# 82magnolia/piccolo

Measured on AMD Instinct MI355X. Metric: candidate-poses/s, higher is better.
Workload: dtype f32

## Files before the change

piccolo_amd/csrc/pcl_gd.hip:

```cpp
#include <stdlib.h>
#include <string.h>

#include "pcl_gd_device.h"
#include "pcl_gd_state.h"
#include "pcl_host.h"
#include "pcl_timer.h"

#define PCL_GD_MAX_IMAGES 64


__global__ void pcl_pose_setup_kernel(const float* __restrict__ trans, const float* __restrict__ rot, int B, PclPoseRec* recs)
{
    int b = blockIdx.x * blockDim.x + threadIdx.x;
    if (b >= B) return;
    float p[6] = {trans[3 * b], trans[3 * b + 1], trans[3 * b + 2], rot[3 * b], rot[3 * b + 1], rot[3 * b + 2]};
    pcl_write_pose_rec(&recs[b], p);
}

template <int G>
__global__ void __launch_bounds__(PCL_GD_THREADS) pcl_finish_kernel(const float* __restrict__ partials, int nchunks, int B,
                                                                    const PclPoseRec* __restrict__ recs,
                                                                    const float* __restrict__ rot, int with_grad,
                                                                    float* __restrict__ result)
{
    __shared__ double rows_sh[(PCL_GD_THREADS / 16) * 2 * G][4];
    __shared__ double sums_sh[G][PCL_NACC];
    pcl_reduce_group<G>(partials, nchunks, blockIdx.x, threadIdx.x, rows_sh, sums_sh);
    if (threadIdx.x < G) {
        const int b = blockIdx.x * G + threadIdx.x;
        double s[PCL_NACC];
        for (int q = 0; q < PCL_NACC; q++) s[q] = sums_sh[threadIdx.x][q];
        float loss, g[6] = {0, 0, 0, 0, 0, 0};
        if (with_grad) {
            double sy, cy, sp, cp;
            sincos((double)rot[3 * b], &sy, &cy);
            sincos((double)rot[3 * b + 1], &sp, &cp);
            pcl_chain_rule(s, recs[b].R, sy, cy, sp, cp, loss, g);
        } else loss = (float)s[0] / (float)s[1];
        float* r = result + (int64_t)b * PCL_RESULT_STRIDE;
        r[0] = loss; r[1] = (float)s[1];
        for (int k = 0; k < 6; k++) r[2 + k] = g[k];
    }
}

static int gd_depth_grid(int64_t n, int H, int W, int depth_h, int depth_w, float tau, int stride_in, PclDepthGrid* g, int* stride)
{
    if (depth_h < 0 || depth_w < 0 || (depth_h == 0) != (depth_w == 0) || !(tau >= 0.f) || stride_in < 0 || stride_in > 64) return PCL_EINVAL;
    int st = stride_in;
    if (depth_h == 0) {
        int rc = pcl_depth_default(n, H, W, stride_in, &depth_h, &depth_w, nullptr, &st);
        if (rc) return rc;
    } else if (st == 0) st = 1;
    if (stride) *stride = st;
    if (depth_h < 2 || depth_w < 2 || depth_h >= (1 << 24) || depth_w >= (1 << 24) || (int64_t)depth_h * depth_w > ((int64_t)1 << 28)) return PCL_EINVAL;
    *g = pcl_make_depth_grid(depth_h, depth_w, tau);
    return 0;
}

struct GdLossWs { PclPoseRec* recs; float* partials; uint32_t* zbuf; };
static size_t gd_loss_layout(void* base, int64_t n, int B, const PclDepthGrid* grid, GdLossWs* w)
{
    PclCarve c{(char*)base, 0};
    w->recs = (PclPoseRec*)c.raw((size_t)B * sizeof(PclPoseRec));
    w->partials = (float*)c.raw(pcl_partials_bytes(n, B));
    w->zbuf = nullptr;
    if (grid) {
        c.off = pcl_align256(c.off);
        w->zbuf = (uint32_t*)c.raw(pcl_depth_zbuf_bytes(B, grid->Hd, grid->Wd));
    }
    return c.off;
}

extern "C" size_t pcl_loss_workspace_bytes(int64_t n, int B)
{
    GdLossWs w;
    return n <= 0 || B <= 0 ? 0 : gd_loss_layout(nullptr, n, B, nullptr, &w);
}

extern "C" size_t pcl_loss_depth_workspace_bytes(int64_t n, int B, int H, int W, int depth_h, int depth_w, int depth_stride)
{
    PclDepthGrid g;
    GdLossWs w;
    if (n <= 0 || B <= 0 || gd_depth_grid(n, H, W, depth_h, depth_w, 0.f, depth_stride, &g, nullptr)) return 0;
    return gd_loss_layout(nullptr, n, B, &g, &w);
// ... 140 lines not shown
    GdRunWs w;
    if (hyper_host->depth_mask && gd_depth_grid(n, H, W, hyper_host->depth_h, hyper_host->depth_w, 0.f, hyper_host->depth_stride, &g, nullptr)) return 0;
    return gd_run_layout(nullptr, n, B, sets, hyper_host->depth_mask ? &g : nullptr, &w);
}

extern "C" int pcl_gd_init(void* state, const float* trans, const float* rot, int B, const pcl_gd_hyper* hyper_host, void* stream)
{
    if (!state || !trans || !rot || !hyper_host || B <= 0) return PCL_EINVAL;
    const int sets = gd_sets(B, hyper_host);
    if (sets < 0) return PCL_EINVAL;
    hipLaunchKernelGGL(pcl_gd_init_kernel, dim3((B + 255) / 256), dim3(256), 0, (hipStream_t)stream, gd_poses(state),
                       gd_recs(state, B), gd_recs(state, B, 1), trans, rot, B, hyper_host->lr, sets > 1 ? B / sets : 0);
    PCL_LAUNCH_CHECK();
    return 0;
}

static int gd_fuse_limit(const pcl_gd_hyper* hyper_host)
{
    if (hyper_host && hyper_host->fuse < 0) return 0;
    return PCL_KNOB(GD_FUSE_BLOCKS, 1024);
}

extern "C" int pcl_gd_plan_hyper(int64_t n, int B, const pcl_gd_hyper* hyper_host, int* nchunks_host, int* poses_per_block_host, int* fused_host)
{
    if (n <= 0 || n > PCL_MAX_POINTS || B <= 0) return PCL_EINVAL;
    const int sets = gd_sets(B, hyper_host);
    if (sets < 0) return PCL_EINVAL;
    if (nchunks_host) *nchunks_host = pcl_plan_nchunks(n, B, sets);
    if (poses_per_block_host) *poses_per_block_host = pcl_plan_G(n, B, sets);
    const bool depth = hyper_host && hyper_host->depth_mask;
    if (fused_host) *fused_host = (!depth && pcl_plan_nblocks(n, B, sets) <= gd_fuse_limit(hyper_host)) ? 1 : 0;
    return 0;
}

extern "C" int pcl_gd_plan(int64_t n, int B, int* nchunks_host, int* poses_per_block_host, int* fused_host)
{
    return pcl_gd_plan_hyper(n, B, nullptr, nchunks_host, poses_per_block_host, fused_host);
}

static bool gd_run_args_ok(const void* what, const void* pano, const void* state, const pcl_gd_hyper* hyper_host, const void* workspace, int H, int W,
                           int num_iter)
{
    return what && pano && state && hyper_host && workspace && H > 0 && W > 0 && num_iter >= 0 &&
           (hyper_host->mode == PCL_GD_SEQUENTIAL || hyper_host->mode == PCL_GD_BATCH);
}

template <class Before, class Loss, class Epilogue>
static int gd_chain_loop(void* state, int B, bool fused, const float* box, const pcl_gd_hyper* hyper_host, int num_iter, float* loss_history,
                         float* const partials2[2], PclTimer* tm, hipStream_t s, Before before, Loss loss, Epilogue epilogue)
{
    auto history = [&](int it) { return loss_history ? loss_history + (int64_t)it * B : nullptr; };
    for (int it = 0; it < num_iter; it++) {
        int rc = before(it);
        if (rc) return rc;
        bool timed;
        hipError_t e = pcl_timer_begin(tm, it, s, &timed);
        if (e != hipSuccess) return (int)e;
        if (fused && it > 0) {
            const int cin = (it - 1) & 1, cout = it & 1;
            PclFuseArgs f;
            f.partials_in = partials2[cin]; f.st_in = gd_poses(state, B, cin); f.recs_in = gd_recs(state, B, cin);
            f.st_out = gd_poses(state, B, cout); f.recs_out = gd_recs(state, B, cout);
            f.box = box; f.factor = hyper_host->factor; f.patience = (int)hyper_host->patience; f.mode = (int)hyper_host->mode;
            f.loss_out = history(it - 1);
            rc = loss(it, f.recs_in, partials2[cout], &f);
        } else {
            rc = loss(it, gd_recs(state, B), partials2[0], nullptr);
        }
        if (rc) return rc;
        if (timed && (e = pcl_timer_end(tm, s)) != hipSuccess) return (int)e;
        if (!fused) {
            epilogue(0, partials2[0], history(it));
            PCL_LAUNCH_CHECK();
        }
    }
    if (fused && num_iter > 0) {
        const int last = num_iter > 1 ? (num_iter - 1) & 1 : 0;
        epilogue(last, partials2[last], history(num_iter - 1));
        PCL_LAUNCH_CHECK();
    }
    return 0;
}

static int gd_run(const float* cloud, const float* weights, int wsets, int64_t n, const void* pano, int pano_format, int H, int W, void* state, int B,
                  const float* box, const pcl_gd_hyper* hyper_host, int num_iter, float* loss_history, void* workspace, size_t workspace_bytes,
                  void* timer, void* stream)
{
    if (!gd_run_args_ok(cloud, pano, state, hyper_host, workspace, H, W, num_iter) || !box || n <= 0 || n > PCL_MAX_POINTS || B <= 0) return PCL_EINVAL;
    const int sets = gd_sets(B, hyper_host);
    if (sets < 0 || (sets > 1 && pcl_cloud_sets_bytes(n, sets) == 0)) return PCL_EINVAL;
    const int psets = wsets > 0 ? wsets : sets;
    hipStream_t s = (hipStream_t)stream;
    const bool depth_on = hyper_host->depth_mask != 0;
    PclDepthLook look;
    look.zbuf = nullptr;
    int zstride = 1;
    if (depth_on) {
        int rcg = gd_depth_grid(n, H, W, hyper_host->depth_h, hyper_host->depth_w, hyper_host->depth_tau, hyper_host->depth_stride, &look.grid, &zstride);
        if (rcg) return rcg;
        look.zclear_vec4 = (int64_t)(pcl_depth_zbuf_bytes(B, look.grid.Hd, look.grid.Wd) / 16);
    }
    GdRunWs w;
    if (workspace_bytes < gd_run_layout(workspace, n, B, psets, depth_on ? &look.grid : nullptr, &w)) return PCL_EWORKSPACE;
    static const int pingpong_env = PCL_KNOB(ZPINGPONG, 1);
    const int nchunks = pcl_plan_nchunks(n, B, psets);
    static const int flip_env = PCL_KNOB(FLIP, 1);
    const int xcd_bit = hyper_host->images > 1 && n * 24 <= ((int64_t)6 << 20) ? 2 : 0;
    const bool fused = !depth_on && pcl_plan_nblocks(n, B, psets) <= gd_fuse_limit(hyper_host);
    const int G = pcl_plan_G(n, B, psets);
    return gd_chain_loop(
        state, B, fused, box, hyper_host, num_iter, loss_history, w.partials, (PclTimer*)timer, s,
        [&](int it) {
            if (!depth_on) return 0;
            const int set = pingpong_env ? (it & 1) : 0;
            look.zbuf = w.zbuf[set];
            look.zclear = pingpong_env ? w.zbuf[set ^ 1] : nullptr;
            return pcl_launch_zbuffers(cloud, n, gd_recs(state, B), B, look.grid, zstride, w.zbuf[set], it == 0 || !pingpong_env, s);
        },
        [&](int it, const PclPoseRec* recs, float* partials, const PclFuseArgs* fuse) {
            return pcl_launch_loss(cloud, n, pano, pano_format, H, W, recs, B, true, nullptr, partials, s, (flip_env ? (it & 1) : 0) | xcd_bit, fuse,
                                   depth_on ? &look : nullptr, sets, weights, wsets);
        },
        [&](int copy_in, const float* partials, float* loss_out) {
            pcl_with_G<4>(G, [&](auto g) {
                constexpr int GG = decltype(g)::value;
                hipLaunchKernelGGL(pcl_gd_epilogue_kernel<GG>, dim3(B / GG), dim3(PCL_GD_THREADS), 0, s, partials, nchunks, gd_poses(state, B, copy_in),
                                   gd_recs(state, B, copy_in), gd_poses(state, B, 0), gd_recs(state, B, 0), box, hyper_host->factor,
                                   (int)hyper_host->patience, (int)hyper_host->mode, loss_out);
            });
        });
}

extern "C" int pcl_gd_run(const float* cloud, int64_t n, const void* pano, int pano_format, int H, int W, void* state, int B,
                          const float* box, const pcl_gd_hyper* hyper_host, int num_iter, float* loss_history,
                          void* workspace, size_t workspace_bytes, void* timer, void* stream)
{
    return gd_run(cloud, nullptr, 0, n, pano, pano_format, H, W, state, B, box, hyper_host, num_iter, loss_history, workspace, workspace_bytes, timer, stream);
}

extern "C" int pcl_gd_run_weighted(const float* cloud, const float* weights, int64_t n, const void* pano, int pano_format, int H, int W, void* state,
                                   int B, const float* box, const pcl_gd_hyper* hyper_host, int num_iter, float* loss_history, void* workspace,
                                   size_t workspace_bytes, void* timer, void* stream)
{
    if (!weights || !hyper_host || hyper_host->depth_mask || hyper_host->color_sets > 1) return PCL_EINVAL;
    if (!pcl_weighted_plan_ok(n, B)) return PCL_EINVAL;
    return gd_run(cloud, weights, 0, n, pano, pano_format, H, W, state, B, box, hyper_host, num_iter, loss_history, workspace, workspace_bytes, timer, stream);
}


static bool gd_weight_sets_ok(int64_t n, int B, int nsets, const pcl_gd_hyper* hyper_host)
{
    if (!hyper_host || n <= 0 || n > PCL_MAX_POINTS || B <= 0 || nsets < 1 || B % nsets) return false;
    if (hyper_host->depth_mask || hyper_host->color_sets < 0 || (hyper_host->color_sets > 1 && hyper_host->color_sets != nsets)) return false;
    if (hyper_host->color_sets > 1 && pcl_cloud_sets_bytes(n, nsets) == 0) return false;
    const int G = pcl_plan_G(n, B, nsets);
    return G <= 2 && (B / nsets) % G == 0;
}

extern "C" size_t pcl_gd_weight_sets_workspace_bytes(int64_t n, int B, int nsets, const pcl_gd_hyper* hyper_host)
{
    GdRunWs w;
    return gd_weight_sets_ok(n, B, nsets, hyper_host) ? gd_run_layout(nullptr, n, B, nsets, nullptr, &w) : 0;
}

extern "C" int pcl_gd_plan_weight_sets(int64_t n, int B, int nsets, const pcl_gd_hyper* hyper_host, int* nchunks_host, int* poses_per_block_host,
                                       int* fused_host)
{
    if (!gd_weight_sets_ok(n, B, nsets, hyper_host)) return PCL_EINVAL;
    if (nchunks_host) *nchunks_host = pcl_plan_nchunks(n, B, nsets);
    if (poses_per_block_host) *poses_per_block_host = pcl_plan_G(n, B, nsets);
    if (fused_host) *fused_host = pcl_plan_nblocks(n, B, nsets) <= gd_fuse_limit(hyper_host) ? 1 : 0;
    return 0;
}

extern "C" int pcl_gd_init_weight_sets(void* state, const float* trans, const float* rot, int B, int nsets, const pcl_gd_hyper* hyper_host, void* stream)
{
    if (!state || !trans || !rot || !hyper_host || B <= 0 || nsets < 1 || B % nsets) return PCL_EINVAL;
    if (hyper_host->depth_mask || hyper_host->color_sets < 0 || (hyper_host->color_sets > 1 && hyper_host->color_sets != nsets)) return PCL_EINVAL;
    hipLaunchKernelGGL(pcl_gd_init_kernel, dim3((B + 255) / 256), dim3(256), 0, (hipStream_t)stream, gd_poses(state), gd_recs(state, B),
                       gd_recs(state, B, 1), trans, rot, B, hyper_host->lr, B / nsets);
    PCL_LAUNCH_CHECK();
    return 0;
}

extern "C" int pcl_gd_run_weight_sets(const float* cloud, const float* weights, int nsets, int64_t n, const void* pano, int pano_format, int H, int W,
                                      void* state, int B, const float* box, const pcl_gd_hyper* hyper_host, int num_iter, float* loss_history,
                                      void* workspace, size_t workspace_bytes, void* timer, void* stream)
{
    if (!gd_weight_sets_ok(n, B, nsets, hyper_host)) return PCL_EINVAL;
    return gd_run(cloud, weights, nsets, n, pano, pano_format, H, W, state, B, box, hyper_host, num_iter, loss_history, workspace, workspace_bytes, timer,
                  stream);
}


template <int G>
__global__ void __launch_bounds__(PCL_GD_THREADS) pcl_gd_epilogue_rooms_kernel(const float* __restrict__ partials, const PclRoomTable* __restrict__ rooms,
                                                                               int ngroups, const PclGdPose* st_in, const PclPoseRec* recs_in,
                                                                               PclGdPose* st_out, PclPoseRec* recs_out, double factor, int patience,
                                                                               int mode, float* loss_out)
{
    __shared__ double rows_sh[(PCL_GD_THREADS / 16) * 2 * G][4];
    __shared__ double sums_sh[G][PCL_NACC];
    const int r = (int)blockIdx.x / ngroups, grp = (int)blockIdx.x - r * ngroups;
    const PclRoomRec* rm = rooms->rec + r;
    const int pose0 = pcl_rfl(rm->group0) * G, nchunks = pcl_rfl(rm->nchunks);
    const float* part = partials + (long long)pcl_rfl64((unsigned long long)rm->partials);
    const float* box = (const float*)pcl_rfl64(rm->box);
    pcl_gd_finish_group<G, false>(part, nchunks, grp, threadIdx.x, st_in + pose0, recs_in + pose0, st_out + pose0, recs_out + pose0, true, box, factor,
                                  patience, mode, loss_out ? loss_out + pose0 : nullptr, rows_sh, sums_sh, nullptr);
}

__global__ void pcl_gd_rooms_table_kernel(PclRoomTable t, PclRoomTable* dst)
{
// ... 408 lines not shown
```

piccolo_amd/csrc/pcl_host.h:

```cpp
#pragma once
#include <type_traits>

#include "pcl_device.h"

struct PclFuseArgs;
struct PclRoomTable;
struct PclDepthTable;

size_t pcl_partials_bytes(int64_t n, int B, int sets = 1);
int pcl_plan_nchunks(int64_t n, int B, int sets = 1);
int pcl_plan_nblocks(int64_t n, int B, int sets = 1);
int pcl_plan_G(int64_t n, int B, int sets = 1);
void pcl_plan_room_images(int64_t n, int per_image, int nimages, int* G, int* ngroups, int* nchunks, int* seg_len, int* steps_base, int* steps_rem);
void pcl_plan_for_groups(int64_t n, int ngroups, int* nchunks, int* seg_len, int* steps_base, int* steps_rem);
int pcl_launch_loss(const float* cloud, int64_t n, const void* pano, int pano_format, int H, int W, const PclPoseRec* poses, int B, bool grad,
                    const uint8_t* visible, float* partials, hipStream_t s, int flip, const PclFuseArgs* fuse, const PclDepthLook* depth,
                    int color_sets = 1, const float* weights = nullptr, int wsets = 0);
static inline bool pcl_weighted_plan_ok(int64_t n, int B) { return n > 0 && n <= PCL_MAX_POINTS && B > 0 && pcl_plan_G(n, B) <= 2; }
int pcl_launch_loss_rooms(const PclRoomTable* rooms, const void* pano, int pano_format, int H, int W, const PclPoseRec* poses, int B, int G,
                          int ngroups, int nblk, float* partials, hipStream_t s, int flip, const PclFuseArgs* fuse, int color_sets = 1,
                          const PclDepthTable* dtab = nullptr, const PclDepthLook* depth = nullptr);

size_t pcl_depth_zbuf_bytes(int B, int Hd, int Wd);
int pcl_launch_zbuffers(const float* cloud, int64_t n, const PclPoseRec* poses, int B, const PclDepthGrid& g, int zstride, uint32_t* zbuf, bool fill,
                        hipStream_t s);

static inline size_t pcl_align256(size_t v) { return (v + 255) & ~(size_t)255; }
struct PclCarve {
    char* base;
    size_t off;
    void* raw(size_t bytes) { void* p = base ? base + off : nullptr; off += bytes; return p; }
    void* take(size_t bytes) { return raw(pcl_align256(bytes)); }
};

template <class F>
static inline void pcl_with_flag(bool v, F&& f)
{
    if (v) return f(std::true_type{});
    f(std::false_type{});
}

template <int MAXG, class F>
static inline void pcl_with_G(int G, F&& f)
{
    if constexpr (MAXG >= 4) {
        if (G == 4) return f(std::integral_constant<int, 4>{});
    }
    if (G == 2) return f(std::integral_constant<int, 2>{});
    f(std::integral_constant<int, 1>{});
}
```

piccolo_amd/csrc/pcl_loss.hip:

```cpp
#include <stdlib.h>

#include "pcl_gd_device.h"
#include "pcl_host.h"
#include "pcl_sample_device.h"

struct PclLossArgs {
    const float* cloud;
    int64_t n, stride;
    const void* pano;
    PclDims dims;
    const PclPoseRec* poses;
    int B;
    const uint8_t* visible;
    const uint32_t* zbuf;
    PclDepthGrid dgrid;
    pcl_i4* zclear;
    int zclear_per_block;
    int64_t zclear_total;
    float* partials;
    int nchunks;
    int ngroups;
    int flip;
    int seg_len;
    int xcd_groups;
// ... 421 lines not shown
{
    PclPlan p = pcl_plan(n, 2 * ngroups);
    static const int chunks_env = PCL_KNOB(TRIM_CHUNKS, 0);
    int auto_chunks = 0;
    const int64_t per_chunk = n <= 2000000 ? 8192 : 16384;
    if (chunks_env < 8 && n > 64 * per_chunk) auto_chunks = (int)((n + per_chunk - 1) / per_chunk);
    if (chunks_env >= 8 || auto_chunks) {
        int64_t steps = (n + PCL_STEP - 1) / PCL_STEP, want = (((chunks_env >= 8 ? chunks_env : auto_chunks) + 7) / 8) * 8;
        if (want > steps) want = ((steps + 7) / 8) * 8;
        p.nchunks = (int)want; p.steps_base = (int)(steps / want); p.steps_rem = (int)(steps % want);
        static const int runs_env = PCL_KNOB(TRIM_RUNS, 0);
        int cpx = p.nchunks / 8, runs = runs_env < 1 || runs_env > cpx ? cpx : runs_env;
        while (cpx % runs) runs--;
        p.seg_len = cpx / runs;
    }
    *nchunks = p.nchunks; *seg_len = p.seg_len; *steps_base = p.steps_base; *steps_rem = p.steps_rem;
}


template <int MAXG, class F>
static inline void pcl_with_G_fmt(int G, int pano_format, F&& f)
{
    pcl_with_G<MAXG>(G, [&](auto g) {
        if (pano_format == PCL_PANO_U8) f(g, std::integral_constant<int, PCL_PANO_U8>{});
        else if (pano_format == PCL_PANO_F16) f(g, std::integral_constant<int, PCL_PANO_F16>{});
        else f(g, std::integral_constant<int, PCL_PANO_F32>{});
    });
}

static int pcl_loss_args(PclLossArgs* a, const void* pano, int pano_format, int H, int W, const PclPoseRec* poses, int B, float* partials, int flip,
                         int color_sets)
{
    if (pano_format != PCL_PANO_F32 && pano_format != PCL_PANO_U8 && pano_format != PCL_PANO_F16) return PCL_EINVAL;
    if ((int64_t)(H + 2) * (W + 2) * pcl_texel_bytes(pano_format) >= ((int64_t)1 << 31)) return PCL_EINVAL;
    *a = PclLossArgs{};
    a->pano = pano; a->dims = pcl_make_dims(H, W, pano_format);
    a->poses = poses; a->B = B; a->partials = partials;
    a->flip = flip & 1; a->color_sets = color_sets > 1 ? color_sets : 1;
    return 0;
}

static void pcl_loss_args_zclear(PclLossArgs* a, const PclDepthLook* depth, int64_t nblk)
{
    a->zclear = (pcl_i4*)depth->zclear;
    a->zclear_total = depth->zclear_vec4;
    a->zclear_per_block = (int)((depth->zclear_vec4 + nblk - 1) / nblk);
}

int pcl_launch_loss_rooms(const PclRoomTable* rooms, const void* pano, int pano_format, int H, int W, const PclPoseRec* poses, int B, int G,
                          int ngroups, int nblk, float* partials, hipStream_t s, int flip, const PclFuseArgs* fuse, int color_sets,
                          const PclDepthTable* dtab, const PclDepthLook* depth)
{
    PclLossArgs a;
    int rc = pcl_loss_args(&a, pano, pano_format, H, W, poses, B, partials, flip, color_sets);
    if (rc) return rc;
    if ((G != 1 && G != 2) || nblk <= 0) return PCL_EINVAL;
    a.ngroups = ngroups;
    if (dtab) {
        if (fuse || !depth || !depth->zbuf || !depth->zclear) return PCL_EINVAL;
        a.zbuf = depth->zbuf;
        pcl_loss_args_zclear(&a, depth, nblk);
    }
    const bool sets = color_sets > 1;
    const dim3 grid(nblk), blk(PCL_BLOCK);
    pcl_with_G_fmt<2>(G, pano_format, [&](auto g, auto fmt) {
        constexpr int GG = decltype(g)::value, FMT = decltype(fmt)::value;
        if (dtab) {
            if (sets) hipLaunchKernelGGL((pcl_loss_rooms_sets_depth_kernel<GG, FMT>), grid, blk, 0, s, a, rooms, dtab);
            else hipLaunchKernelGGL((pcl_loss_rooms_depth_kernel<GG, FMT>), grid, blk, 0, s, a, rooms, dtab);
        } else if (sets) {
            if (fuse) hipLaunchKernelGGL((pcl_loss_fused_rooms_sets_kernel<GG, FMT>), grid, blk, 0, s, a, *fuse, rooms);
            else hipLaunchKernelGGL((pcl_loss_rooms_sets_kernel<GG, FMT>), grid, blk, 0, s, a, rooms);
        } else {
            if (fuse) hipLaunchKernelGGL((pcl_loss_fused_rooms_kernel<GG, FMT>), grid, blk, 0, s, a, *fuse, rooms);
            else hipLaunchKernelGGL((pcl_loss_rooms_kernel<GG, FMT>), grid, blk, 0, s, a, rooms);
        }
    });
    PCL_LAUNCH_CHECK();
    return 0;
}

int pcl_launch_loss(const float* cloud, int64_t n, const void* pano, int pano_format, int H, int W, const PclPoseRec* poses,
                    int B, bool grad, const uint8_t* visible, float* partials, hipStream_t s, int flip, const PclFuseArgs* fuse,
                    const PclDepthLook* depth, int color_sets, const float* weights, int wsets)
{
    PclLossArgs a;
    int rc = pcl_loss_args(&a, pano, pano_format, H, W, poses, B, partials, flip, color_sets);
    if (rc) return rc;
    if (n > PCL_MAX_POINTS) return PCL_EINVAL;
    const bool sets = color_sets > 1;
    if (sets && (B % color_sets || !grad || visible || depth || pcl_cloud_sets_bytes(n, color_sets) == 0)) return PCL_EINVAL;
    if (wsets > 0 && (B % wsets || !grad || visible || depth || (sets && color_sets != wsets))) return PCL_EINVAL;
    if (weights && (visible || depth || (wsets > 0 ? pcl_plan_G(n, B, wsets) > 2 : sets || !pcl_weighted_plan_ok(n, B)))) return PCL_EINVAL;
    const PclPlan p = pcl_plan_sets(n, B, wsets > 0 ? wsets : color_sets);
    const int nblk = p.nchunks * p.ngroups;
    a.cloud = cloud; a.n = n; a.stride = pcl_cloud_stride(n);
    a.visible = visible;
    if (depth) {
        if (visible || !depth->zbuf || depth->grid.Hd <= 0 || depth->grid.Wd <= 0) return PCL_EINVAL;
        if ((int64_t)B * depth->grid.Hd * depth->grid.Wd * 4 >= ((int64_t)1 << 32)) return PCL_EINVAL;
        a.zbuf = depth->zbuf; a.dgrid = depth->grid;
        if (depth->zclear) pcl_loss_args_zclear(&a, depth, nblk);
    }
    a.nchunks = p.nchunks; a.ngroups = p.ngroups; a.seg_len = p.seg_len; a.steps_base = p.steps_base; a.steps_rem = p.steps_rem;
    static const int xg_env = PCL_KNOB(XCD_GROUPS, -1);
    a.xcd_groups = ((flip & 2) != 0 || xg_env == 1) && xg_env != 0 && p.ngroups % 8 == 0 ? 1 : 0;
    const int vis = depth ? 2 : visible != nullptr ? 1 : 0;
    if (fuse && (!grad || vis)) return PCL_EINVAL;
    const dim3 grid(nblk), blk(PCL_BLOCK);
    if (weights && wsets > 0) {
        pcl_with_G_fmt<2>(p.G, pano_format, [&](auto g, auto fmt) {
            constexpr int GG = decltype(g)::value, FMT = decltype(fmt)::value;
            pcl_with_flag(sets, [&](auto cs) {
                constexpr bool CSS = decltype(cs)::value;
                if (fuse) hipLaunchKernelGGL((pcl_loss_fused_wsets_kernel<GG, FMT, CSS>), grid, blk, 0, s, a, *fuse, weights);
                else hipLaunchKernelGGL((pcl_loss_wsets_kernel<GG, FMT, CSS>), grid, blk, 0, s, a, weights);
            });
        });
        PCL_LAUNCH_CHECK();
        return 0;
    }
    if (weights) {
        pcl_with_G_fmt<2>(p.G, pano_format, [&](auto g, auto fmt) {
            constexpr int GG = decltype(g)::value, FMT = decltype(fmt)::value;
            if (fuse) hipLaunchKernelGGL((pcl_loss_fused_wt_kernel<GG, FMT>), grid, blk, 0, s, a, *fuse, weights);
            else if (grad) hipLaunchKernelGGL((pcl_loss_wt_kernel<GG, true, FMT>), grid, blk, 0, s, a, weights);
            else hipLaunchKernelGGL((pcl_loss_wt_kernel<GG, false, FMT>), grid, blk, 0, s, a, weights);
        });
        PCL_LAUNCH_CHECK();
        return 0;
    }
    pcl_with_G_fmt<4>(p.G, pano_format, [&](auto g, auto fmt) {
        constexpr int GG = decltype(g)::value, FMT = decltype(fmt)::value;
        if (sets) {
            if (fuse) hipLaunchKernelGGL((pcl_loss_fused_sets_kernel<GG, FMT>), grid, blk, 0, s, a, *fuse);
            else hipLaunchKernelGGL((pcl_loss_sets_kernel<GG, FMT>), grid, blk, 0, s, a);
        } else if (fuse) hipLaunchKernelGGL((pcl_loss_fused_kernel<GG, FMT>), grid, blk, 0, s, a, *fuse);
        else if (grad) {
            if (vis == 2) hipLaunchKernelGGL((pcl_loss_kernel<GG, true, 2, FMT>), grid, blk, 0, s, a);
            else if (vis) hipLaunchKernelGGL((pcl_loss_kernel<GG, true, 1, FMT>), grid, blk, 0, s, a);
            else hipLaunchKernelGGL((pcl_loss_kernel<GG, true, 0, FMT>), grid, blk, 0, s, a);
        } else {
            if (vis == 2) hipLaunchKernelGGL((pcl_loss_kernel<GG, false, 2, FMT>), grid, blk, 0, s, a);
            else if (vis) hipLaunchKernelGGL((pcl_loss_kernel<GG, false, 1, FMT>), grid, blk, 0, s, a);
            else hipLaunchKernelGGL((pcl_loss_kernel<GG, false, 0, FMT>), grid, blk, 0, s, a);
        }
    });
    PCL_LAUNCH_CHECK();
    return 0;
}
```

piccolo_amd/ops.py:

```python
import ctypes

import torch

from . import _lib


class _Experiment:
    pano_fmt = None
    trim_fmt = None
    gd_graph = None
    verify_levels = False


EXPERIMENT = _Experiment()

F32 = torch.float32


_GPU_SEEN = False


def device():
    global _GPU_SEEN
    if not _GPU_SEEN:
# ... 702 lines not shown


class ColorTemplate:

    def __init__(self, rgb):
        lib = _lib.load()
        rgb = _dev(rgb).reshape(-1, 3)
        self.n = int(rgb.shape[0])
        self.data = torch.empty(3, self.n, dtype=F32, device=rgb.device)
        nws = lib.pcl_color_template_workspace_bytes(self.n)
        ws = _bytes(nws)
        _lib.check(lib.pcl_color_template_build(_ptr(rgb), self.n, _ptr(self.data), _ptr(ws), nws, _stream()),
                   "pcl_color_template_build")


def color_match(img, template):
    lib = _lib.load()
    known = _known_levels(img)
    img = _dev(img)
    H, W = int(img.shape[0]), int(img.shape[1])
    out = torch.empty_like(img)
    flag = torch.zeros(1, dtype=torch.int32, device=img.device)
    nws = lib.pcl_color_workspace_bytes()
    ws = _bytes(nws)
    _lib.check(lib.pcl_color_match(_ptr(img), H, W, _ptr(template.data), template.n, _ptr(out), _ptr(flag), _ptr(ws), nws,
                                   _stream()), "pcl_color_match")
    if not known and int(flag.item()):
        raise ValueError("color_match: the panorama must hold levels k/255 (an image file's uint8 / 255); "
                         "found a non-black pixel channel in between")
    return out


def color_mod(img, rgb, num_bins=256):
    lib = _lib.load()
    img, rgb = _dev(img), _dev(rgb).reshape(-1, 3)
    H, W = int(img.shape[0]), int(img.shape[1])
    out_img, out_rgb = torch.empty_like(img), torch.empty_like(rgb)
    nws = lib.pcl_color_workspace_bytes()
    ws = _bytes(nws)
    _lib.check(lib.pcl_color_mod(_ptr(img), H, W, _ptr(rgb), int(rgb.shape[0]), int(num_bins), _ptr(out_img), _ptr(out_rgb),
                                 _ptr(ws), nws, _stream()), "pcl_color_mod")
    return out_img, out_rgb


def histogram(img, mask, channels, normalize=True, eps=0.0):
    lib = _lib.load()
    img = _dev(img).reshape(-1, 3)
    mask = _dev(mask != 0, torch.uint8).reshape(-1)
    c0, c1, c2 = (int(c) for c in channels)
    nws = lib.pcl_histogram_workspace_bytes(c0, c1, c2)
    if nws == 0:
        raise ValueError("histogram: bad bin counts %r" % (channels,))
    ws = _bytes(nws)
    hist = torch.empty(c0 * c1 * c2, dtype=F32, device=img.device)
    _lib.check(lib.pcl_histogram(_ptr(img), _ptr(mask), int(img.shape[0]), c0, c1, c2, int(bool(normalize)), float(eps),
                                 _ptr(hist), _ptr(ws), nws, _stream()), "pcl_histogram")
    return hist


def histogram_intersection(h1, h2):
    lib = _lib.load()
    h1, h2 = _dev(h1), _dev(h2)
    B, nbins = int(h1.shape[0]), int(h1.shape[1])
    out = torch.empty(B, dtype=F32, device=h1.device)
    _lib.check(lib.pcl_histogram_intersection(_ptr(h1), _ptr(h2), B, nbins, _ptr(out), _stream()), "pcl_histogram_intersection")
    return out


def quantile_box(xyz, q):
    lib = _lib.load()
    xyz = _dev(xyz)
    box = torch.empty(6, dtype=F32, device=xyz.device)
    ws = _bytes(lib.pcl_quantile_workspace_bytes())
    _lib.check(lib.pcl_quantile_box(_ptr(xyz), int(xyz.shape[0]), float(q), _ptr(box), _ptr(ws), _stream()), "pcl_quantile_box")
    return box


def _checked(name, *args):
    _lib.check(getattr(_lib.load(), name)(*args), name)


def _gd_hyper(lr, patience, factor, batch_mode, fuse, depth=None, color_sets=0):
    dh, dw, tau, st = depth or (0, 0, 0.0, 0)
    return _lib.GdHyper(float(lr), float(factor), int(patience), _lib.GD_BATCH if batch_mode else _lib.GD_SEQUENTIAL, 1 if depth else 0, float(tau),
                        int(dh), int(dw), int(st), -1 if fuse is False else 0, 0, int(color_sets))


class _GdEngine:

    def run_graph(self, num_iter):
        cache = self.__dict__.setdefault("_graphs", {})
        key = (num_iter,) + tuple(self._graph_key())
        g = cache.get(key)
        if g is None:
            g = torch.cuda.CUDAGraph()
            side = torch.cuda.Stream(device=self.state.device)
            side.wait_stream(torch.cuda.current_stream())
            with torch.cuda.stream(side):
                with torch.cuda.graph(g, stream=side):
                    self.run(num_iter)
            torch.cuda.current_stream().wait_stream(side)
            cache[key] = g
        g.replay()

    def _graph_key(self):
        return ()

    def _name_panos(self, panos):
        I = len(panos)
        if I <= 0 or self.B % I:
            raise ValueError("set_pano_groups: %d candidates do not split into %d images" % (self.B, I))
        for p in panos:
            if (p.H, p.W, p.fmt) != (self.pano.H, self.pano.W, self.pano.fmt):
                raise ValueError("all panoramas of a launch must share size and texel format")
        self._panos = list(panos)
        arr = (ctypes.c_uint64 * I)(*[p.data.data_ptr() for p in panos])
        _lib.check(_lib.load().pcl_gd_set_pano_groups(_ptr(self.state), arr, I, self.B // I, _stream()), "pcl_gd_set_pano_groups")

    def winners(self, groups, leaf_trans=None, leaf_rot=None):
        if groups <= 0 or self.B % groups:
            raise ValueError("winner: %d candidates do not split into %d images" % (self.B, groups))
        out = torch.empty(groups, 16, dtype=F32, device=self.state.device)
        for t in (leaf_trans, leaf_rot):
            if t is not None and not (t.is_cuda and t.dtype == F32 and t.is_contiguous() and t.numel() == 3 * self.B):
                raise ValueError("winner: leaf buffers must be contiguous float32 GPU tensors of B x 3")
        _lib.check(_lib.load().pcl_gd_winner(_ptr(self.state), groups, self.B // groups, _ptr(out), _ptr(leaf_trans), _ptr(leaf_rot), _stream()),
                   "pcl_gd_winner")
        return out

    def result(self):
        out = torch.empty(self.B, _lib.GD_RESULT_STRIDE, dtype=F32, device=self.state.device)
        _lib.check(_lib.load().pcl_gd_result(_ptr(self.state), self.B, _ptr(out), _stream()), "pcl_gd_result")
        return out

    def pruned(self, keep, leaf_trans=None, leaf_rot=None):
        child = self._smaller(int(keep))
        return child, self.prune_into(child, leaf_trans, leaf_rot)

    def prune_into(self, child, leaf_trans=None, leaf_rot=None):
        groups = self._groups()
        if type(child) is not type(self) or child is self or child.B <= 0 or child.B % groups or child.B > self.B or not self._same_problem(child):
            raise ValueError("prune: the smaller engine must be one of the same class, clouds and groups with at most as many candidates")
        for t in (leaf_trans, leaf_rot):
            if t is not None and not (t.is_cuda and t.dtype == F32 and t.is_contiguous() and t.numel() == 3 * self.B):
                raise ValueError("prune: leaf buffers must be contiguous float32 GPU tensors of B x 3")
        if self.B // groups > _lib.GD_PRUNE_MAX:
            raise ValueError("prune: at most %d candidates per group" % _lib.GD_PRUNE_MAX)
        survivors = torch.empty(child.B, dtype=torch.int32, device=self.state.device)
        _lib.check(_lib.load().pcl_gd_prune(_ptr(self.state), groups, self.B // groups, child.B // groups, _ptr(child.state), _ptr(survivors),
                                            _ptr(leaf_trans), _ptr(leaf_rot), _stream()), "pcl_gd_prune")
        child.hyper.images = self.hyper.images
        for name in ("_panos", "_pano_table"):
            if name in self.__dict__:
                setattr(child, name, self.__dict__[name])
        return survivors


def _copy_hyper(h):
    c = _lib.GdHyper()
    ctypes.memmove(ctypes.byref(c), ctypes.byref(h), ctypes.sizeof(c))
    return c


class GradientDescent(_GdEngine):

    def __init__(self, cloud, pano, trans, rot, box, lr=0.1, patience=5, factor=0.9, batch_mode=True, depth_mask=False,
                 depth_tau=None, depth_res=None, depth_stride=None, fuse=None, weight_sets=0):
        lib = _lib.load()
# ... 424 lines not shown
```

Baseline: 3534.

## Split GD loss and epilogue across two streams by pose-group halves

When the non-fused, non-depth GD path has enough blocks, the pose groups are split into two halves. Each half's loss and epilogue kernels run on its own stream (the main stream plus a per-device side stream), joined with events, and on the first iteration the side stream's start is staggered. The goal is to let one half's epilogue tail overlap with the other half's loss work instead of serializing behind it. This adds event, stream and mutex overhead, is disabled during graph capture, and adds new fuse modes to force or disable the split.

```diff
diff --git a/piccolo_amd/csrc/pcl_gd.hip b/piccolo_amd/csrc/pcl_gd.hip
--- a/piccolo_amd/csrc/pcl_gd.hip
+++ b/piccolo_amd/csrc/pcl_gd.hip
@@ -1,5 +1,7 @@
 #include <stdlib.h>
 #include <string.h>
+
+#include <mutex>
 
 #include "pcl_gd_device.h"
 #include "pcl_gd_state.h"
@@ -306,6 +308,50 @@
     return 0;
 }
 
+#define PCL_GD_MAX_DEVICES 64
+struct GdSide {
+    std::mutex mu;
+    bool ready = false;
+    hipStream_t stream = nullptr;
+    hipEvent_t fork = nullptr, stagger = nullptr, join = nullptr;
+};
+static GdSide gd_sides[PCL_GD_MAX_DEVICES];
+
+static GdSide* gd_side_acquire(hipStream_t s)
+{
+    hipStreamCaptureStatus cap = hipStreamCaptureStatusActive;
+    if (hipStreamIsCapturing(s, &cap) != hipSuccess || cap != hipStreamCaptureStatusNone) { (void)hipGetLastError(); return nullptr; }
+    int dev = -1;
+    if (hipGetDevice(&dev) != hipSuccess || dev < 0 || dev >= PCL_GD_MAX_DEVICES) return nullptr;
+    GdSide* sd = &gd_sides[dev];
+    sd->mu.lock();
+    if (!sd->ready) {
+        hipStreamCaptureMode mode = hipStreamCaptureModeRelaxed;
+        bool ok = hipThreadExchangeStreamCaptureMode(&mode) == hipSuccess;
+        if (ok) {
+            ok = hipStreamCreateWithFlags(&sd->stream, hipStreamNonBlocking) == hipSuccess &&
+                 hipEventCreateWithFlags(&sd->fork, hipEventDisableTiming) == hipSuccess &&
+                 hipEventCreateWithFlags(&sd->stagger, hipEventDisableTiming) == hipSuccess &&
+                 hipEventCreateWithFlags(&sd->join, hipEventDisableTiming) == hipSuccess;
+            (void)hipThreadExchangeStreamCaptureMode(&mode);
+        }
+        if (!ok) {
+            (void)hipGetLastError();
+            if (sd->fork) (void)hipEventDestroy(sd->fork);
+            if (sd->stagger) (void)hipEventDestroy(sd->stagger);
+            if (sd->join) (void)hipEventDestroy(sd->join);
+            if (sd->stream) (void)hipStreamDestroy(sd->stream);
+            sd->stream = nullptr; sd->fork = sd->stagger = sd->join = nullptr;
+            sd->mu.unlock();
+            return nullptr;
+        }
+        sd->ready = true;
+    }
+    return sd;
+}
+
+static int gd_split_min_blocks() { return PCL_KNOB(GD_SPLIT_BLOCKS, 896); }
+
 static int gd_run(const float* cloud, const float* weights, int wsets, int64_t n, const void* pano, int pano_format, int H, int W, void* state, int B,
                   const float* box, const pcl_gd_hyper* hyper_host, int num_iter, float* loss_history, void* workspace, size_t workspace_bytes,
                   void* timer, void* stream)
@@ -332,7 +378,31 @@
     const int xcd_bit = hyper_host->images > 1 && n * 24 <= ((int64_t)6 << 20) ? 2 : 0;
     const bool fused = !depth_on && pcl_plan_nblocks(n, B, psets) <= gd_fuse_limit(hyper_host);
     const int G = pcl_plan_G(n, B, psets);
-    return gd_chain_loop(
+    const int ngroups = B / G;
+    const int gA = ngroups / 2;
+    GdSide* side = nullptr;
+    if (!fused && !depth_on && num_iter > 0 && ngroups >= 2 && hyper_host->fuse != -2 &&
+        (hyper_host->fuse == -3 || (int64_t)gA * nchunks >= gd_split_min_blocks()))
+        side = gd_side_acquire(s);
+    if (side) {
+        hipError_t e = hipEventRecord(side->fork, s);
+        if (e == hipSuccess) e = hipStreamWaitEvent(side->stream, side->fork, 0);
+        if (e != hipSuccess) { side->mu.unlock(); return (int)e; }
+    }
+    auto loss_range = [&](int it, const PclPoseRec* recs, float* partials, hipStream_t st, int g0, int g1) {
+        return pcl_launch_loss(cloud, n, pano, pano_format, H, W, recs, B, true, nullptr, partials, st, (flip_env ? (it & 1) : 0) | xcd_bit, nullptr, nullptr,
+                               sets, weights, wsets, g0, g1);
+    };
+    auto epilogue_range = [&](const float* partials, float* loss_out, hipStream_t st, int g0, int g1) {
+        pcl_with_G<4>(G, [&](auto g) {
+            constexpr int GG = decltype(g)::value;
+            const int64_t p0 = (int64_t)g0 * GG;
+            hipLaunchKernelGGL(pcl_gd_epilogue_kernel<GG>, dim3(g1 - g0), dim3(PCL_GD_THREADS), 0, st, partials + (int64_t)g0 * nchunks * GG * PCL_NACC, nchunks,
+                               gd_poses(state, B, 0) + p0, gd_recs(state, B, 0) + p0, gd_poses(state, B, 0) + p0, gd_recs(state, B, 0) + p0, box,
+                               hyper_host->factor, (int)hyper_host->patience, (int)hyper_host->mode, loss_out ? loss_out + p0 : nullptr);
+        });
+    };
+    int rc = gd_chain_loop(
         state, B, fused, box, hyper_host, num_iter, loss_history, w.partials, (PclTimer*)timer, s,
         [&](int it) {
             if (!depth_on) return 0;
@@ -342,10 +412,25 @@
             return pcl_launch_zbuffers(cloud, n, gd_recs(state, B), B, look.grid, zstride, w.zbuf[set], it == 0 || !pingpong_env, s);
         },
         [&](int it, const PclPoseRec* recs, float* partials, const PclFuseArgs* fuse) {
-            return pcl_launch_loss(cloud, n, pano, pano_format, H, W, recs, B, true, nullptr, partials, s, (flip_env ? (it & 1) : 0) | xcd_bit, fuse,
-                                   depth_on ? &look : nullptr, sets, weights, wsets);
+            if (!side)
+                return pcl_launch_loss(cloud, n, pano, pano_format, H, W, recs, B, true, nullptr, partials, s, (flip_env ? (it & 1) : 0) | xcd_bit, fuse,
+                                       depth_on ? &look : nullptr, sets, weights, wsets);
+            int rcl;
+            if (it == 0 && gA >= 2) {
+                if ((rcl = loss_range(it, recs, partials, s, 0, gA / 2))) return rcl;
+                hipError_t e = hipEventRecord(side->stagger, s);
+                if (e == hipSuccess) e = hipStreamWaitEvent(side->stream, side->stagger, 0);
+                if (e != hipSuccess) return (int)e;
+                if ((rcl = loss_range(it, recs, partials, s, gA / 2, gA))) return rcl;
+            } else if ((rcl = loss_range(it, recs, partials, s, 0, gA))) return rcl;
+            return loss_range(it, recs, partials, side->stream, gA, ngroups);
         },
         [&](int copy_in, const float* partials, float* loss_out) {
+            if (side) {
+                epilogue_range(partials, loss_out, s, 0, gA);
+                epilogue_range(partials, loss_out, side->stream, gA, ngroups);
+                return;
+            }
             pcl_with_G<4>(G, [&](auto g) {
                 constexpr int GG = decltype(g)::value;
                 hipLaunchKernelGGL(pcl_gd_epilogue_kernel<GG>, dim3(B / GG), dim3(PCL_GD_THREADS), 0, s, partials, nchunks, gd_poses(state, B, copy_in),
@@ -353,6 +438,13 @@
                                    (int)hyper_host->patience, (int)hyper_host->mode, loss_out);
             });
         });
+    if (side) {
+        hipError_t e = hipEventRecord(side->join, side->stream);
+        if (e == hipSuccess) e = hipStreamWaitEvent(s, side->join, 0);
+        side->mu.unlock();
+        if (!rc && e != hipSuccess) rc = (int)e;
+    }
+    return rc;
 }
 
 extern "C" int pcl_gd_run(const float* cloud, int64_t n, const void* pano, int pano_format, int H, int W, void* state, int B,
diff --git a/piccolo_amd/csrc/pcl_host.h b/piccolo_amd/csrc/pcl_host.h
--- a/piccolo_amd/csrc/pcl_host.h
+++ b/piccolo_amd/csrc/pcl_host.h
@@ -15,7 +15,7 @@
 void pcl_plan_for_groups(int64_t n, int ngroups, int* nchunks, int* seg_len, int* steps_base, int* steps_rem);
 int pcl_launch_loss(const float* cloud, int64_t n, const void* pano, int pano_format, int H, int W, const PclPoseRec* poses, int B, bool grad,
                     const uint8_t* visible, float* partials, hipStream_t s, int flip, const PclFuseArgs* fuse, const PclDepthLook* depth,
-                    int color_sets = 1, const float* weights = nullptr, int wsets = 0);
+                    int color_sets = 1, const float* weights = nullptr, int wsets = 0, int g0 = 0, int g1 = -1);
 static inline bool pcl_weighted_plan_ok(int64_t n, int B) { return n > 0 && n <= PCL_MAX_POINTS && B > 0 && pcl_plan_G(n, B) <= 2; }
 int pcl_launch_loss_rooms(const PclRoomTable* rooms, const void* pano, int pano_format, int H, int W, const PclPoseRec* poses, int B, int G,
                           int ngroups, int nblk, float* partials, hipStream_t s, int flip, const PclFuseArgs* fuse, int color_sets = 1,
diff --git a/piccolo_amd/csrc/pcl_loss.hip b/piccolo_amd/csrc/pcl_loss.hip
--- a/piccolo_amd/csrc/pcl_loss.hip
+++ b/piccolo_amd/csrc/pcl_loss.hip
@@ -527,7 +527,7 @@
 
 int pcl_launch_loss(const float* cloud, int64_t n, const void* pano, int pano_format, int H, int W, const PclPoseRec* poses,
                     int B, bool grad, const uint8_t* visible, float* partials, hipStream_t s, int flip, const PclFuseArgs* fuse,
-                    const PclDepthLook* depth, int color_sets, const float* weights, int wsets)
+                    const PclDepthLook* depth, int color_sets, const float* weights, int wsets, int g0, int g1)
 {
     PclLossArgs a;
     int rc = pcl_loss_args(&a, pano, pano_format, H, W, poses, B, partials, flip, color_sets);
@@ -537,7 +537,15 @@
     if (sets && (B % color_sets || !grad || visible || depth || pcl_cloud_sets_bytes(n, color_sets) == 0)) return PCL_EINVAL;
     if (wsets > 0 && (B % wsets || !grad || visible || depth || (sets && color_sets != wsets))) return PCL_EINVAL;
     if (weights && (visible || depth || (wsets > 0 ? pcl_plan_G(n, B, wsets) > 2 : sets || !pcl_weighted_plan_ok(n, B)))) return PCL_EINVAL;
-    const PclPlan p = pcl_plan_sets(n, B, wsets > 0 ? wsets : color_sets);
+    PclPlan p = pcl_plan_sets(n, B, wsets > 0 ? wsets : color_sets);
+    if (g1 >= 0) {
+        if (g0 < 0 || g1 <= g0 || g1 > p.ngroups || !grad || fuse || visible || depth) return PCL_EINVAL;
+        a.poses = poses + (int64_t)g0 * p.G;
+        a.partials = partials + (int64_t)g0 * p.nchunks * p.G * PCL_NACC;
+        a.B = (g1 - g0) * p.G;
+        p.ngroups = g1 - g0;
+        p.seg_len = pcl_xcd_seg_len(p.nchunks, (int64_t)p.nchunks * p.ngroups);
+    }
     const int nblk = p.nchunks * p.ngroups;
     a.cloud = cloud; a.n = n; a.stride = pcl_cloud_stride(n);
     a.visible = visible;
diff --git a/piccolo_amd/ops.py b/piccolo_amd/ops.py
--- a/piccolo_amd/ops.py
+++ b/piccolo_amd/ops.py
@@ -808,8 +808,16 @@
 
 def _gd_hyper(lr, patience, factor, batch_mode, fuse, depth=None, color_sets=0):
     dh, dw, tau, st = depth or (0, 0, 0.0, 0)
+    if fuse is None or fuse is True:
+        fz = 0
+    elif fuse is False:
+        fz = -1
+    elif isinstance(fuse, int) and -3 <= fuse <= 0:
+        fz = int(fuse)
+    else:
+        raise ValueError("fuse: None, True, False or pcl_gd_hyper.fuse's 0, -1, -2, -3, not %r" % (fuse,))
     return _lib.GdHyper(float(lr), float(factor), int(patience), _lib.GD_BATCH if batch_mode else _lib.GD_SEQUENTIAL, 1 if depth else 0, float(tau),
-                        int(dh), int(dw), int(st), -1 if fuse is False else 0, 0, int(color_sets))
+                        int(dh), int(dw), int(st), fz, 0, int(color_sets))
 
 
 class _GdEngine:
```

Measured after the change: 3632 (median of 6 runs). 1.03x the previous value.
